# keras-team/keras-rs

Hardware: AMD Instinct MI355X
Metric: embedding lookups/sec + DCN fwd+bwd step time, 26-table DLRM batch 65 536 (higher is better)
Workload: dtype bf16; 1 GPU; C3 DLRM-small: 26 tables x 1000000 rows x 128 (bf16), global batch 65536, multi-hot ml_perf lengths (sum L = 214), uniform ids, DotInteraction(F=27) + 3 x FeatureCross(d=3456, projection=512), fused Adagrad on tables; global_batch=65536, parallelism=single GPU

## Files before the change

include/krs.h:

```cpp
#ifndef KRS_H_
#define KRS_H_

#include <stddef.h>
#include <stdint.h>

#ifdef __cplusplus
extern "C" {
#endif

#define KRS_VERSION 100

typedef enum krs_status {
  KRS_OK = 0,
  KRS_ERR_INVALID = -1,
  KRS_ERR_UNSUPPORTED = -2,
  KRS_ERR_LAUNCH = -3,
  KRS_ERR_WORKSPACE = -4
} krs_status;

typedef enum krs_dtype { KRS_F32 = 0, KRS_BF16 = 1 } krs_dtype;
typedef enum krs_itype { KRS_I32 = 0, KRS_I64 = 1 } krs_itype;

typedef enum krs_combiner { KRS_SUM = 0, KRS_MEAN = 1, KRS_SQRTN = 2 } krs_combiner;

// ... 87 lines not shown

int krs_embed_bag_bwd_fused_ftrl(const krs_table* tables, int n_tables,
                                 const krs_feature* feats, int n_feats,
                                 const float* weights, const float* bag_scale,
                                 const void* grad, int grad_dtype, int64_t grad_ld,
                                 int batch, int dim, int table_dtype, int64_t nnz,
                                 float learning_rate_power, float l1, float l2, float beta,
                                 const void* workspace, void* stream);

int krs_embed_bag_bwd_fused_adam_dyn(const krs_table* tables, int n_tables,
                                     const krs_feature* feats, int n_feats,
                                     const float* weights, const float* bag_scale,
                                     const void* grad, int grad_dtype, int64_t grad_ld,
                                     int batch, int dim, int table_dtype, int64_t nnz,
                                     float beta_1, float beta_2, float epsilon, const float* bias_correction_dev,
                                     const void* workspace, void* stream);

int krs_store_f32(void* dst, int64_t stride_bytes, const float* values_host, int count, void* stream);

int krs_embed_bag_bwd_sparse(const krs_feature* feats, int n_feats,
                             const float* weights, const float* bag_scale,
                             const void* grad, int grad_dtype, int64_t grad_ld,
                             int batch, int dim, int64_t nnz,
                             const void* workspace,
                             int64_t* unique_rows, float* row_grads, int64_t* n_unique,
                             void* stream);

typedef struct krs_gemm_epilogue {
  const float* bias;
  int32_t act;
  float diag_scale;
  const void* x0;
  const void* x;
  int64_t ldx;
  void* u_out;
  int64_t ldu;
  const void* r;
  int64_t ldr;
  float beta;
} krs_gemm_epilogue;

int krs_gemm(const void* a, int64_t lda, int a_is_km,
             const void* b, int64_t ldb, int b_is_nk,
             void* c, int64_t ldc,
             int64_t m, int64_t n, int64_t k,
             int in_dtype, int out_dtype,
             const krs_gemm_epilogue* epilogue,
             void* workspace, size_t workspace_bytes, void* stream);
size_t krs_gemm_workspace_bytes(int64_t m, int64_t n, int64_t k, int a_is_km);

size_t krs_gemm_cross_bwd_workspace_bytes(int64_t m, int64_t n);
int krs_gemm_cross_bwd(const void* a, int64_t lda, const void* bt, int64_t ldb,
                       const void* r, int64_t ldr, float beta,
                       void* g_out, int64_t ldg,
                       const void* x0, const void* u, void* dz, void* dx0, int64_t ld, int dx0_accumulate,
                       const void* u_upper, int fold_direct, float* dbias, int64_t m, int64_t n, int64_t k, int act, int dtype,
                       void* workspace, size_t workspace_bytes, void* stream);
int krs_gemm_dense_bwd(const void* a, int64_t lda, const void* bt, int64_t ldb, void* g_out, int64_t ldg,
                       const void* y, void* dz, int64_t ld, float* dbias, int64_t m, int64_t n, int64_t k, int act,
                       int dtype, void* workspace, size_t workspace_bytes, void* stream);
enum { KRS_CROSS_BWD_NONE = 0, KRS_CROSS_BWD_TWO_CALL = 1, KRS_CROSS_BWD_PP64 = 2, KRS_CROSS_BWD_PP256 = 3 };
int krs_gemm_cross_bwd_last_route(int* epilogue);

enum {
  KRS_GEMM_KERNEL_NONE = 0, KRS_GEMM_KERNEL_GENERIC = 1, KRS_GEMM_KERNEL_MFMA = 2, KRS_GEMM_KERNEL_GLDS = 3,
  KRS_GEMM_KERNEL_TN_GLDS = 4, KRS_GEMM_KERNEL_PP256 = 5, KRS_GEMM_KERNEL_PP256_KSTRIDED = 6, KRS_GEMM_KERNEL_PP64 = 7,
  KRS_GEMM_KERNEL_THIN = 8, KRS_GEMM_KERNEL_ROWDOT = 9, KRS_GEMM_KERNEL_SMALLK = 10
};
enum { KRS_GEMM_REDUCE_NONE = 0, KRS_GEMM_REDUCE_SCALAR = 1, KRS_GEMM_REDUCE_VEC4 = 2, KRS_GEMM_REDUCE_VEC8 = 3 };
typedef struct krs_gemm_route {
  int32_t kernel;
  int32_t splits;
  int32_t reduce;
  int32_t epilogue;
  int32_t ep_vec;
  int32_t thin_width;
  int32_t thin_is_a;
} krs_gemm_route;
int krs_gemm_last_route(krs_gemm_route* route);

enum { KRS_GEMM_OPT_PIPELINE = 0 };
int krs_gemm_set_option(int key, int value);

enum { KRS_EMBED_OPT_PLAN = 2, KRS_EMBED_OPT_HOTROWS = 3 };
int krs_embed_set_option(int key, int value);

size_t krs_colsum_workspace_bytes(int64_t m, int64_t n);
int krs_cross_epilogue_fwd(const void* u, const void* x0, const void* x, void* y,
                           int64_t m, int64_t n, int64_t ld, float diag_scale,
                           int dtype, void* stream);
int krs_cross_epilogue_bwd(const void* g, const void* u, const void* x0, const void* x,
                           void* du, void* dx0, int dx0_accumulate, void* dxd,
                           float* dbias,
                           int64_t m, int64_t n, int64_t ld, float diag_scale, int act,
                           int dtype, void* workspace, size_t workspace_bytes, void* stream);

int krs_cast_transpose(const void* src, int64_t rows, int64_t cols, int64_t ld_src, int src_dtype,
                       void* dst, int64_t ld_dst, void* dst_t, int64_t ld_dst_t, int dst_dtype,
                       void* stream);
int krs_cast_transpose_many(int count, const void* const* srcs, const int64_t* rows, const int64_t* cols,
                            int src_dtype, void* const* dsts, void* const* dst_ts, int dst_dtype, void* stream);

int krs_dense_act_bwd(const void* g, int64_t ld_g, const void* y, int64_t ld_y, void* dz, int64_t ld_dz,
                      float* dbias, int64_t m, int64_t n, int act, int dtype, void* workspace,
                      size_t workspace_bytes, void* stream);

int krs_dense_adagrad(float* const* params, const float* const* grads, float* const* accs,
                      const int64_t* sizes, int count, float lr, float eps, void* stream);

int krs_colsum(const void* a, int64_t lda, int64_t m, int64_t n, int dtype,
               float* out, void* workspace, size_t workspace_bytes, void* stream);

int krs_dot_interaction_fwd(const void* const* feats, const int64_t* ld, int n_feats,
                            int64_t batch, int dim, int dtype,
                            int self_interaction, int skip_gather,
                            void* out, int64_t out_ld, void* stream);
int krs_dot_interaction_bwd(const void* const* feats, const int64_t* ld, int n_feats,
                            int64_t batch, int dim, int dtype,
                            int self_interaction, int skip_gather,
                            const void* grad_out, int64_t grad_ld,
                            void* const* grad_feats, const int64_t* grad_feat_ld,
                            void* stream);
int krs_dot_interaction_bwd_accumulate(const void* const* feats, const int64_t* ld, int n_feats,
                                       int64_t batch, int dim, int dtype,
                                       int self_interaction, int skip_gather,
                                       const void* grad_out, int64_t grad_ld,
                                       void* const* grad_feats, const int64_t* grad_feat_ld,
                                       uint64_t accumulate_mask, void* stream);

size_t krs_mod_bucketize_workspace_bytes(int64_t nnz, int n_shards);
int krs_mod_bucketize(const void* ids, int id_type, int64_t nnz, int n_shards,
                      void* local_ids, int32_t* perm, int64_t* bucket_counts,
                      void* workspace, size_t workspace_bytes, void* stream);

#define KRS_BCE_MAX_BLOCKS 64
int krs_bce_fwd_bwd(const void* pred, int pred_dtype, const float* labels, int64_t n, float epsilon,
                    float grad_scale, float* loss, void* dpred, float* partials, void* stream);

typedef struct krs_shard_feature {
  int64_t ids_base;
  int64_t comp_off;
  int32_t hot;
  int32_t combiner;
  int32_t vocab;
  int32_t reserved;
} krs_shard_feature;

size_t krs_shard_route_workspace_bytes(int64_t nnz, int64_t n_bags, int n_shards);
int krs_shard_route(const krs_shard_feature* feats, const krs_shard_feature* feats_host, int n_feats,
                    const void* ids, int id_type, const void* offsets, int offset_type,
                    const float* weights, int64_t nnz, int batch, int n_shards, int emit_weights,
                    int32_t* packed, int32_t* seg_bag, int32_t* seg_grow, int32_t* bag_seg,
                    int64_t* counts, int32_t* err_flag,
                    void* workspace, size_t workspace_bytes, void* stream);
size_t krs_shard_unpack_workspace_bytes(int64_t total_segments);
int krs_shard_unpack(const int32_t* packed, int n_sources, const int64_t* lookups, const int64_t* segments,
                     int weighted, int32_t* rows, float* w, int32_t* offsets,
                     void* workspace, size_t workspace_bytes, void* stream);
int krs_shard_combine(const void* partials, const int32_t* bag_seg, int batch, int n_feats, int n_shards,
                      int dim, int dtype, void* out, int64_t out_ld, void* stream);
int64_t krs_shard_static_block_words(int64_t cap_lookups, int64_t cap_segments, int emit_weights);
int krs_shard_route_static(const krs_shard_feature* feats, const krs_shard_feature* feats_host, int n_feats,
                           const void* ids, int id_type, const void* offsets, int offset_type,
                           const float* weights, int64_t nnz, int batch, int n_shards, int emit_weights,
                           int64_t cap_lookups, int64_t cap_segments,
                           int32_t* packed, int32_t* seg_bag, int32_t* seg_grow, int32_t* bag_seg,
                           int64_t* counts, int32_t* err_flag,
// ... 73 lines not shown
```

keras_rs_amd/csrc/embed_bag_fwd.hip:

```cpp
#include <cstdlib>

#include "krs_common.h"

namespace krs {
namespace {

typedef uint32_t u32x4 __attribute__((ext_vector_type(4)));
typedef float f32x4 __attribute__((ext_vector_type(4)));
constexpr int NT = 2;

struct EmbedFwdParams {
  const krs_table* tables;
  const krs_feature* feats;
  int n_feats;
  const void* ids;
  int id64;
  const void* offsets;
  int off64;
  const float* weights;
  int batch;
  int dim;
  void* out;
  int64_t out_ld;
  float* bag_scale;
// ... 462 lines not shown
    sw2 = fmaf(w, w, sw2);
  }
  const int comb = ft.combiner;
  const float den = comb == KRS_MEAN ? sw : (comb == KRS_SQRTN ? sqrtf(sw2) : 1.0f);
  for (int c = sub; c < p.dim; c += lpr) {
    float acc = 0.0f;
    for (int64_t q = s; q < e; ++q) {
      const int64_t id = ld_index(p.ids, p.id64, q);
      if (id < 0 || id >= tb.vocab) {
        oob = 1;
        continue;
      }
      const float w = p.weights ? p.weights[q] : 1.0f;
      acc = fmaf(w, ld_elem(tb.weights, table_dtype, id * p.dim + c), acc);
    }
    if (comb != KRS_SUM) acc = den == 0.0f ? 0.0f : acc / den;
    st_elem(p.out, out_dtype, (int64_t)b * p.out_ld + ft.out_col + c, acc);
  }
  if (p.bag_scale && sub == 0)
    p.bag_scale[bag] = comb == KRS_SUM ? 1.0f : (den == 0.0f ? 0.0f : 1.0f / den);
  if (oob && p.err_flag && sub == 0) atomicOr(p.err_flag, KRS_FLAG_ID_OUT_OF_RANGE);
}

int g_hot_rows = 0;

template <typename TT, typename OT, int LPR>
int launch_vec(const EmbedFwdParams& p, bool one_hot, bool stream, hipStream_t st) {
  constexpr int G = 64 / LPR;
  if (one_hot) {
    if constexpr (sizeof(TT) == sizeof(OT)) {
      const bool rows_ok = p.n_feats <= kRowsMaxFeats &&
                           ((reinterpret_cast<uintptr_t>(p.out) | (uintptr_t)(p.out_ld * sizeof(OT))) & 15) == 0;
      if (rows_ok) {
        const int64_t blocks = ceil_div(ceil_div((int64_t)p.batch * p.n_feats, 64), 4);
        if (blocks > 0x7fffffffLL) return fail(KRS_ERR_UNSUPPORTED, "embed_bag_fwd: grid too large");
        hipLaunchKernelGGL((embed_gather_hot1_rows<TT, LPR, 16>), dim3((unsigned)blocks), dim3(256), 0, st, p);
        KRS_CHECK_LAUNCH("embed_gather_hot1_rows");
        return KRS_OK;
      }
    }
    const int64_t blocks = ceil_div(ceil_div(p.batch, 64) * p.n_feats, 4);
    if (blocks > 0x7fffffffLL) return fail(KRS_ERR_UNSUPPORTED, "embed_bag_fwd: grid too large");
    hipLaunchKernelGGL((embed_gather_hot1<TT, OT, LPR, 16>), dim3((unsigned)blocks), dim3(256), 0, st, p);
    KRS_CHECK_LAUNCH("embed_gather_hot1");
    return KRS_OK;
  }
  const int64_t waves_per_feat = ceil_div(p.batch, (int64_t)G * p.bpg);
  const int64_t blocks = ceil_div(waves_per_feat * p.n_feats, 4);
  if (blocks == 0) return KRS_OK;
  if (blocks > 0x7fffffffLL) return fail(KRS_ERR_UNSUPPORTED, "embed_bag_fwd: grid too large");
#define KRS_K1_LAUNCH(W, S) \
  hipLaunchKernelGGL((embed_bag_fwd_vec<TT, OT, LPR, W, S>), dim3((unsigned)blocks), dim3(256), 0, st, p)
  if constexpr (sizeof(TT) == 2 && sizeof(OT) == 2 && LPR == 16) {
    if (g_hot_rows > 0 && !p.weights && (int64_t)p.dim * 2 == LPR * 16) {
      if (g_hot_rows >= 128) {
        if (stream) hipLaunchKernelGGL((embed_bag_fwd_vec<TT, OT, LPR, false, true, 128>), dim3((unsigned)blocks), dim3(256), 0, st, p);
        else hipLaunchKernelGGL((embed_bag_fwd_vec<TT, OT, LPR, false, false, 128>), dim3((unsigned)blocks), dim3(256), 0, st, p);
      } else {
        if (stream) hipLaunchKernelGGL((embed_bag_fwd_vec<TT, OT, LPR, false, true, 64>), dim3((unsigned)blocks), dim3(256), 0, st, p);
        else hipLaunchKernelGGL((embed_bag_fwd_vec<TT, OT, LPR, false, false, 64>), dim3((unsigned)blocks), dim3(256), 0, st, p);
      }
      KRS_CHECK_LAUNCH("embed_bag_fwd_vec (hot rows in LDS)");
      return KRS_OK;
    }
  }
  if (p.weights) { if (stream) KRS_K1_LAUNCH(true, true); else KRS_K1_LAUNCH(true, false); }
  else { if (stream) KRS_K1_LAUNCH(false, true); else KRS_K1_LAUNCH(false, false); }
#undef KRS_K1_LAUNCH
  KRS_CHECK_LAUNCH("embed_bag_fwd_vec");
  return KRS_OK;
}

template <typename TT, typename OT>
int dispatch_lpr(const EmbedFwdParams& p, int row_pieces, bool one_hot, bool stream_mode, hipStream_t stream) {
  if (row_pieces <= 8) return launch_vec<TT, OT, 8>(p, one_hot, stream_mode, stream);
  if (row_pieces <= 16) return launch_vec<TT, OT, 16>(p, one_hot, stream_mode, stream);
  if (row_pieces <= 32) return launch_vec<TT, OT, 32>(p, one_hot, stream_mode, stream);
  return launch_vec<TT, OT, 64>(p, one_hot, stream_mode, stream);
}

}
}

namespace krs { extern int g_plan_variant; }

extern "C" int krs_embed_set_option(int key, int value) {
  if (key == KRS_EMBED_OPT_PLAN) {
    KRS_REQUIRE(value == 0 || value == 1, "krs_embed_set_option: plan variant must be 0 or 1");
    krs::g_plan_variant = value;
    return KRS_OK;
  }
  if (key == KRS_EMBED_OPT_HOTROWS) {
    KRS_REQUIRE(value == 0 || value == 64 || value == 128, "krs_embed_set_option: hot rows must be 0, 64 or 128");
    krs::g_hot_rows = value;
    return KRS_OK;
  }
  return krs::fail(KRS_ERR_INVALID, "krs_embed_set_option: unknown key %d", key);
}

extern "C" int krs_embed_bag_fwd(const krs_table* tables, const krs_feature* feats, int n_feats,
                                 const void* ids, int id_type, const void* offsets, int off_type,
                                 const float* weights, int64_t nnz, int batch, int dim,
                                 int table_dtype, void* out, int out_dtype, int64_t out_ld,
                                 float* bag_scale, int* err_flag, void* stream) {
  using namespace krs;
  KRS_REQUIRE(tables && feats && out, "embed_bag_fwd: null tables/feats/out");
  KRS_REQUIRE(ids || nnz == 0, "embed_bag_fwd: null ids");
  KRS_REQUIRE(n_feats >= 0 && batch >= 0 && dim > 0 && nnz >= 0, "embed_bag_fwd: negative size");
  KRS_REQUIRE((table_dtype == KRS_F32 || table_dtype == KRS_BF16) &&
                  (out_dtype == KRS_F32 || out_dtype == KRS_BF16),
              "embed_bag_fwd: bad dtype");
  KRS_REQUIRE((id_type == KRS_I32 || id_type == KRS_I64) && (off_type == KRS_I32 || off_type == KRS_I64),
              "embed_bag_fwd: bad index type");
  if (n_feats == 0 || batch == 0) return KRS_OK;
  hipStream_t st = reinterpret_cast<hipStream_t>(stream);

  EmbedFwdParams p;
  p.tables = tables; p.feats = feats; p.n_feats = n_feats;
  p.ids = ids; p.id64 = id_type == KRS_I64;
  p.offsets = offsets; p.off64 = off_type == KRS_I64;
  p.weights = weights; p.batch = batch; p.dim = dim;
  p.out = out; p.out_ld = out_ld; p.bag_scale = bag_scale; p.err_flag = err_flag;
  const int64_t n_bags = (int64_t)n_feats * batch;
  const int64_t mean_hot = nnz / n_bags > 0 ? nnz / n_bags : 1;
  int bpg = (int)(32 / mean_hot);
  p.bpg = bpg < 1 ? 1 : (bpg > 16 ? 16 : bpg);
  p.bpg = p.bpg < 1 ? 1 : (p.bpg > 16 ? 16 : p.bpg);

  const int64_t row_bytes = (int64_t)dim * (table_dtype == KRS_BF16 ? 2 : 4);
  if (row_bytes % 16 == 0 && row_bytes <= 1024) {
    const int pieces = (int)(row_bytes / 16);
    const bool one_hot = offsets == nullptr && weights == nullptr && nnz == n_bags;
    const bool stream_mode = nnz < 2 * n_bags;
    if (table_dtype == KRS_F32)
      return out_dtype == KRS_F32 ? dispatch_lpr<float, float>(p, pieces, one_hot, stream_mode, st)
                                  : dispatch_lpr<float, uint16_t>(p, pieces, one_hot, stream_mode, st);
    return out_dtype == KRS_F32 ? dispatch_lpr<uint16_t, float>(p, pieces, one_hot, stream_mode, st)
                                : dispatch_lpr<uint16_t, uint16_t>(p, pieces, one_hot, stream_mode, st);
  }
  int lpr = 1;
  while (lpr < dim && lpr < 64) lpr <<= 1;
  const int64_t blocks = ceil_div(n_bags, 256 / lpr);
  if (blocks > 0x7fffffffLL) return fail(KRS_ERR_UNSUPPORTED, "embed_bag_fwd: grid too large");
  hipLaunchKernelGGL(embed_bag_fwd_generic, dim3((unsigned)blocks), dim3(256), 0, st, p, table_dtype,
                     out_dtype, lpr);
  KRS_CHECK_LAUNCH("embed_bag_fwd_generic");
  return KRS_OK;
}
```

keras_rs_amd/csrc/embed_bag_plan.hip:

```cpp
#include <algorithm>

#include "krs_bag_plan.h"

namespace krs {
int g_plan_variant = 0;
namespace {

namespace rs {
constexpr int kHistThreads = 256, kHistItems = kTile / kHistThreads;
constexpr int kThreads = 512, kWaves = kThreads / 64, kItems = kTile / kThreads;
constexpr int kGenFeats = 256;

struct Gen {
  const krs_table* tables;
  const krs_feature* feats;
  int n_feats;
  const void* ids;
  int id64;
  int batch;
  int* err_flag;
};

struct alignas(16) GenLds {
  uint32_t base[kGenFeats + 1];
  uint32_t hot[kGenFeats];
  uint32_t row_base[kGenFeats];
  uint32_t vocab[kGenFeats];
};
__device__ __forceinline__ void load_gen(const Gen& gen, int64_t nnz, GenLds& g, int n_threads) {
  for (int i = threadIdx.x; i <= gen.n_feats; i += n_threads) {
    if (i < gen.n_feats) {
      const krs_feature ft = gen.feats[i];
      const krs_table tb = gen.tables[ft.table];
      g.base[i] = (uint32_t)ft.ids_base;
      g.hot[i] = (uint32_t)ft.hot;
      g.row_base[i] = (uint32_t)tb.row_base;
      g.vocab[i] = (uint32_t)tb.vocab;
    } else {
      g.base[i] = (uint32_t)nnz;
    }
  }
}
__device__ __forceinline__ int gen_feature(const GenLds& g, int n_feats, uint32_t q) {
  int lo = 0, hi = n_feats;
  while (hi - lo > 1) {
    const int mid = (lo + hi) >> 1;
    if (g.base[mid] <= q) lo = mid; else hi = mid;
  }
  return lo;
}
__device__ __forceinline__ uint64_t gen_value(const Gen& gen, const GenLds& g, int f, uint32_t q) {
  const uint32_t bag = (uint32_t)f * (uint32_t)gen.batch + (q - g.base[f]) / g.hot[f];
  return ((uint64_t)bag << 32) | (uint64_t)q;
}
__device__ __forceinline__ bool generate(const Gen& gen, const GenLds& g, uint32_t q, uint32_t& key, uint64_t& val) {
  const int f = gen_feature(g, gen.n_feats, q);
  const int64_t id = ld_index(gen.ids, gen.id64, q);
  const bool valid = id >= 0 && id < (int64_t)g.vocab[f];
  key = valid ? g.row_base[f] + (uint32_t)id : kInvalidKey;
  val = gen_value(gen, g, f, q);
  return valid;
}

__device__ __forceinline__ int digit_of(uint32_t key, int shift, int bins) { return (int)((key >> shift) & (bins - 1)); }

__device__ __forceinline__ void hist_zero(int (&h)[kMaxBins], int bins) {
  for (int i = threadIdx.x; i < bins; i += kHistThreads) h[i] = 0;
}
__device__ __forceinline__ void hist_add(int (&h)[kMaxBins], uint32_t key, int shift, int bins) {
  atomicAdd(&h[digit_of(key, shift, bins)], 1);
}
__device__ __forceinline__ void hist_finish(const int (&h)[kMaxBins], int bins, int32_t* col, int64_t stride, bool bad,
                                            int* err_flag) {
  if (bad && err_flag) atomicOr(err_flag, KRS_FLAG_ID_OUT_OF_RANGE);
  __syncthreads();
  for (int i = threadIdx.x; i < bins; i += kHistThreads) col[(int64_t)i * stride] = h[i];
}

template <typename V>
struct alignas(16) TileLds {
  uint16_t cnt[kWaves][kMaxBins];
  uint16_t tile_excl[kMaxBins];
  int gbase[kMaxBins];
  uint32_t skey[kTile];
  V sval[kTile];
  int wtot[kWaves];
};
template <typename V>
__device__ __forceinline__ void zero_counts(TileLds<V>& s) {
  for (int i = threadIdx.x; i < kWaves * kMaxBins; i += kThreads) (&s.cnt[0][0])[i] = 0;
}
__device__ __forceinline__ int ballot_rank(uint32_t key, bool live, int shift, int bits, volatile uint16_t* mine,
                                           int lane) {
  const int d = digit_of(key, shift, 1 << bits);
  unsigned long long peers = __ballot(live);
  for (int b = 0; b < bits; ++b) {
    const unsigned long long m = __ballot((d >> b) & 1);
    peers &= ((d >> b) & 1) ? m : ~m;
  }
  int r = 0, c = 0;
  if (live) {
    r = __popcll(peers & ((1ULL << lane) - 1ULL));
    const int leader = __ffsll((long long)peers) - 1;
    if (lane == leader) {
      c = mine[d];
      mine[d] = (uint16_t)(c + __popcll(peers));
    }
    c = __shfl(c, leader, 64);
  }
  __builtin_amdgcn_wave_barrier();
  return c + r;
}
template <typename V>
__device__ __forceinline__ void digit_bases(TileLds<V>& s, int bins, const int32_t* col, int64_t stride) {
  const int lane = threadIdx.x & 63, wave = threadIdx.x >> 6;
  __syncthreads();
  int tot[2], run = 0;
#pragma unroll
  for (int k = 0; k < 2; ++k) {
    const int i = threadIdx.x * 2 + k;
    tot[k] = 0;
    if (i < bins)
      for (int w = 0; w < kWaves; ++w) tot[k] += s.cnt[w][i];
    run += tot[k];
  }
  int x = run;
#pragma unroll
  for (int o = 1; o < 64; o <<= 1) {
    const int y = __shfl_up(x, o, 64);
    if (lane >= o) x += y;
  }
  if (lane == 63) s.wtot[wave] = x;
  __syncthreads();
  int excl = x - run;
  for (int w = 0; w < wave; ++w) excl += s.wtot[w];
#pragma unroll
  for (int k = 0; k < 2; ++k) {
    const int i = threadIdx.x * 2 + k;
    if (i < bins) {
      s.tile_excl[i] = (uint16_t)excl;
      s.gbase[i] = col[(int64_t)i * stride];
      int o = excl;
      for (int w = 0; w < kWaves; ++w) {
        const int t = s.cnt[w][i];
        s.cnt[w][i] = (uint16_t)o;
        o += t;
      }
      excl += tot[k];
    }
  }
  __syncthreads();
}
template <typename V>
__device__ __forceinline__ void stage_tile(TileLds<V>& s, const uint32_t (&key)[kItems], const V (&val)[kItems],
                                           const int (&rank)[kItems], int64_t first, int64_t end, int shift, int bins) {
  const int wave = threadIdx.x >> 6;
#pragma unroll
  for (int it = 0; it < kItems; ++it) {
    if (first + it * 64 < end) {
      const int lp = s.cnt[wave][digit_of(key[it], shift, bins)] + rank[it];
      s.skey[lp] = key[it];
      s.sval[lp] = val[it];
    }
  }
  __syncthreads();
}
template <typename V>
__device__ __forceinline__ int out_slot(const TileLds<V>& s, int i, int d) {
  return s.gbase[d] + (i - (int)s.tile_excl[d]);
}

struct Pass {
  const uint32_t* keys_in;
  const uint64_t* vals_in;
  uint32_t* keys_out;
  uint64_t* vals_out;
  int32_t* counts;
  int64_t nnz;
  int n_tiles;
  int shift, bits;
  Gen gen;
};

template <bool GEN>
__global__ __launch_bounds__(kHistThreads) void hist_kernel(const Pass p) {
  __shared__ int h[kMaxBins];
  __shared__ GenLds g;
  const int bins = 1 << p.bits;
  hist_zero(h, bins);
  if constexpr (GEN) load_gen(p.gen, p.nnz, g, kHistThreads);
  __syncthreads();
  const int64_t base = (int64_t)blockIdx.x * kTile;
  bool bad = false;
  for (int it = 0; it < kHistItems; ++it) {
    const int64_t q = base + it * kHistThreads + threadIdx.x;
    if (q < p.nnz) {
      uint32_t key;
      if constexpr (GEN) {
        uint64_t v;
        bad |= !generate(p.gen, g, (uint32_t)q, key, v);
      } else {
        key = p.keys_in[q];
      }
      hist_add(h, key, p.shift, bins);
    }
  }
  hist_finish(h, bins, p.counts + blockIdx.x, p.n_tiles, bad, p.gen.err_flag);
}

template <bool GEN>
__global__ __launch_bounds__(kThreads) void scatter_kernel(const Pass p) {
  __shared__ TileLds<uint64_t> s;
  __shared__ GenLds g;
  const int bins = 1 << p.bits;
  zero_counts(s);
  if constexpr (GEN) load_gen(p.gen, p.nnz, g, kThreads);
  __syncthreads();
  const int lane = threadIdx.x & 63, wave = threadIdx.x >> 6;
  const int64_t tile0 = (int64_t)blockIdx.x * kTile;
  const int64_t first = tile0 + (int64_t)wave * (kTile / kWaves) + lane;
  uint32_t key[kItems];
  uint64_t val[kItems];
  int rank[kItems];
#pragma unroll
  for (int it = 0; it < kItems; ++it) {
    const int64_t q = first + it * 64;
    const bool live = q < p.nnz;
    key[it] = kInvalidKey;
    val[it] = 0;
    if (live) {
      if constexpr (GEN) {
        generate(p.gen, g, (uint32_t)q, key[it], val[it]);
      } else {
        key[it] = p.keys_in[q];
        val[it] = p.vals_in[q];
      }
    }
    rank[it] = ballot_rank(key[it], live, p.shift, p.bits, s.cnt[wave], lane);
  }
  digit_bases(s, bins, p.counts + blockIdx.x, p.n_tiles);
  stage_tile(s, key, val, rank, first, p.nnz, p.shift, bins);
  const int n_here = (int)min<int64_t>(kTile, p.nnz - tile0);
#pragma unroll
  for (int it = 0; it < kItems; ++it) {
    const int i = it * kThreads + threadIdx.x;
    if (i < n_here) {
      const uint32_t k = s.skey[i];
      const int pos = out_slot(s, i, digit_of(k, p.shift, bins));
      p.keys_out[pos] = k;
      p.vals_out[pos] = s.sval[i];
    }
  }
}

struct Seg {
  int n;
  uint32_t lookup_start[kMaxProb + 1];
  uint32_t tile_start[kMaxProb + 1];
  uint32_t row_base[kMaxProb];
};
struct SegPass {
  const uint32_t* keys_in;
  const uint32_t* pos_in;
  uint32_t* keys_out;
  uint32_t* pos_out;
  uint64_t* vals_out;
  int32_t* counts;
  int64_t nnz;
  int shift, bits, key_bits;
  Gen gen;
  Seg seg;
};
struct SegTile {
  int pr;
  int64_t t0, end;
  int32_t* col;
  uint32_t stride;
};
__device__ __forceinline__ SegTile seg_tile(const SegPass& p, uint32_t tile) {
  const Seg& sg = p.seg;
  int lo = 0, hi = sg.n;
  while (hi - lo > 1) {
    const int mid = (lo + hi) >> 1;
    if (sg.tile_start[mid] <= tile) lo = mid; else hi = mid;
  }
  SegTile t;
  t.pr = lo;
  const uint32_t tl = tile - sg.tile_start[lo];
  t.stride = sg.tile_start[lo + 1] - sg.tile_start[lo];
  t.t0 = (int64_t)sg.lookup_start[lo] + (int64_t)tl * kTile;
  t.end = min<int64_t>(t.t0 + kTile, sg.lookup_start[lo + 1]);
  t.col = p.counts + ((int64_t)1 << p.bits) * sg.tile_start[lo] + tl;
  return t;
}
template <int ITEMS, int STRIDE>
__device__ __forceinline__ bool seg_first_keys(const SegPass& p, const GenLds& g, const SegTile& t, int64_t first,
                                               uint32_t (&key)[ITEMS], uint32_t (&pos)[ITEMS]) {
  int64_t idv[ITEMS];
#pragma unroll
  for (int it = 0; it < ITEMS; ++it) idv[it] = ld_index(p.gen.ids, p.gen.id64, min<int64_t>(first + it * STRIDE, t.end - 1));
  const int f_lo = gen_feature(g, p.gen.n_feats, (uint32_t)t.t0), f_hi = gen_feature(g, p.gen.n_feats, (uint32_t)(t.end - 1));
  bool bad = false;
#pragma unroll
  for (int it = 0; it < ITEMS; ++it) {
    const int64_t q = min<int64_t>(first + it * STRIDE, t.end - 1);
    const int f = f_lo == f_hi ? f_lo : gen_feature(g, p.gen.n_feats, (uint32_t)q);
    const bool valid = idv[it] >= 0 && idv[it] < (int64_t)g.vocab[f];
    key[it] = valid ? (uint32_t)idv[it] : (1u << p.key_bits) - 1u;
    pos[it] = (uint32_t)q;
    bad = bad || (!valid && first + it * STRIDE < t.end);
  }
  return bad;
}

template <bool FIRST>
__global__ __launch_bounds__(kHistThreads) void hist_seg_kernel(const SegPass p) {
  __shared__ int h[kMaxBins];
  __shared__ GenLds g;
  const int bins = 1 << p.bits;
  hist_zero(h, bins);
  if constexpr (FIRST) load_gen(p.gen, p.nnz, g, kHistThreads);
  __syncthreads();
  const SegTile t = seg_tile(p, blockIdx.x);
  const int64_t first = t.t0 + threadIdx.x;
  bool bad = false;
  uint32_t key[kHistItems];
  if constexpr (FIRST) {
    uint32_t pos[kHistItems];
    bad = seg_first_keys<kHistItems, kHistThreads>(p, g, t, first, key, pos);
  } else {
#pragma unroll
    for (int it = 0; it < kHistItems; ++it) key[it] = p.keys_in[min<int64_t>(first + it * kHistThreads, t.end - 1)];
  }
#pragma unroll
  for (int it = 0; it < kHistItems; ++it)
    if (first + it * kHistThreads < t.end) hist_add(h, key[it], p.shift, bins);
  hist_finish(h, bins, t.col, t.stride, bad, p.gen.err_flag);
}

template <bool FIRST, bool LAST>
__global__ __launch_bounds__(kThreads) void scatter_seg_kernel(const SegPass p) {
  __shared__ TileLds<uint32_t> s;
  __shared__ GenLds g;
  const int bins = 1 << p.bits;
  zero_counts(s);
  if constexpr (FIRST || LAST) load_gen(p.gen, p.nnz, g, kThreads);
  __syncthreads();
  const int lane = threadIdx.x & 63, wave = threadIdx.x >> 6;
  const SegTile t = seg_tile(p, blockIdx.x);
  const int64_t first = t.t0 + (int64_t)wave * (kTile / kWaves) + lane;
  uint32_t key[kItems], pos[kItems];
  int rank[kItems];
  if constexpr (FIRST) {
    seg_first_keys<kItems, 64>(p, g, t, first, key, pos);
  } else {
#pragma unroll
    for (int it = 0; it < kItems; ++it) {
      const int64_t q = min<int64_t>(first + it * 64, t.end - 1);
      key[it] = p.keys_in[q];
      pos[it] = p.pos_in[q];
    }
  }
#pragma unroll
  for (int it = 0; it < kItems; ++it) {
    const bool live = first + it * 64 < t.end;
    if (!live) { key[it] = 0xffffffffu; pos[it] = 0; }
    rank[it] = ballot_rank(key[it], live, p.shift, p.bits, s.cnt[wave], lane);
  }
  digit_bases(s, bins, t.col, t.stride);
  stage_tile(s, key, pos, rank, first, t.end, p.shift, bins);
  const int n_here = (int)(t.end - t.t0);
  const uint32_t sentinel = (1u << p.key_bits) - 1u, rb = p.seg.row_base[t.pr];
  int pf_lo = 0, pf_hi = 1;
  if constexpr (LAST) {
    pf_lo = gen_feature(g, p.gen.n_feats, p.seg.lookup_start[t.pr]);
    pf_hi = gen_feature(g, p.gen.n_feats, p.seg.lookup_start[t.pr + 1] - 1);
  }
#pragma unroll
  for (int it = 0; it < kItems; ++it) {
    const int i = it * kThreads + threadIdx.x;
    if (i < n_here) {
      const uint32_t k = s.skey[i], q = s.sval[i];
      const int o = out_slot(s, i, digit_of(k, p.shift, bins));
      if constexpr (LAST) {
        const int f = pf_lo == pf_hi ? pf_lo : gen_feature(g, p.gen.n_feats, q);
        p.keys_out[o] = k == sentinel ? kInvalidKey : rb + k;
        p.vals_out[o] = gen_value(p.gen, g, f, q);
      } else {
        p.keys_out[o] = k;
        p.pos_out[o] = q;
      }
    }
  }
}

inline unsigned key_bits(int64_t n) {
  unsigned bits = 1;
  while (bits < 32 && (1ULL << bits) <= (uint64_t)n) ++bits;
  return bits;
}
struct Schedule {
  int passes;
  int bits[4], shift[4];
};
inline Schedule pass_schedule(unsigned bits) {
  Schedule s;
  s.passes = (int)((bits + kMaxBits - 1) / kMaxBits);
  unsigned done = 0;
  for (int ps = 0; ps < s.passes; ++ps) {
    s.bits[ps] = (int)((bits - done + (s.passes - ps) - 1) / (s.passes - ps));
    s.shift[ps] = (int)done;
    done += (unsigned)s.bits[ps];
  }
  return s;
}
inline Gen make_gen(const krs_table* tables, const krs_feature* feats, int n_feats, const void* ids, int id_type,
                    int batch, int* err_flag) {
  Gen g;
  g.tables = tables; g.feats = feats; g.n_feats = n_feats; g.ids = ids;
  g.id64 = id_type == KRS_I64; g.batch = batch; g.err_flag = err_flag;
  return g;
}
}

struct KeyParams {
  const krs_table* tables;
  const krs_feature* feats;
  int n_feats;
  const void* ids;
  int id64;
  const void* offsets;
  int off64;
  int batch;
  uint32_t* keys;
  uint64_t* vals;
  int* err_flag;
};

__global__ __launch_bounds__(256) void bag_keys_kernel(const KeyParams p) {
  const int64_t bag = (int64_t)blockIdx.x * 16 + (threadIdx.x >> 4);
  const int sub = threadIdx.x & 15;
  if (bag >= (int64_t)p.n_feats * p.batch) return;
  const int f = (int)(bag / p.batch);
  const int b = (int)(bag - (int64_t)f * p.batch);
  const krs_feature ft = p.feats[f];
  const krs_table tb = p.tables[ft.table];
  int64_t s, e;
  if (p.offsets) {
    s = ld_index(p.offsets, p.off64, bag);
    e = ld_index(p.offsets, p.off64, bag + 1);
  } else {
// ... 46 lines not shown
  int c = __popc(seg_head_mask(keys, nnz, (int64_t)blockIdx.x * kSegTile + threadIdx.x * kSegItems));
  for (int o = 32; o; o >>= 1) c += __shfl_down(c, o, 64);
  if ((threadIdx.x & 63) == 0) atomicAdd(&total, c);
  __syncthreads();
  if (threadIdx.x == 0) block_heads[blockIdx.x] = total;
}
__global__ __launch_bounds__(256) void seg_emit_kernel(const uint32_t* keys, int64_t nnz, const int32_t* block_off,
                                                       uint32_t* seg_start, uint32_t* n_seg) {
  __shared__ int wsum[4];
  const int64_t t0 = (int64_t)blockIdx.x * kSegTile + threadIdx.x * kSegItems;
  const uint32_t mask = seg_head_mask(keys, nnz, t0);
  const int c = __popc(mask), lane = threadIdx.x & 63, wave = threadIdx.x >> 6;
  int x = c;
#pragma unroll
  for (int o = 1; o < 64; o <<= 1) {
    const int y = __shfl_up(x, o, 64);
    if (lane >= o) x += y;
  }
  if (lane == 63) wsum[wave] = x;
  __syncthreads();
  uint32_t off = (uint32_t)block_off[blockIdx.x] + (uint32_t)(x - c);
  for (int w = 0; w < wave; ++w) off += (uint32_t)wsum[w];
  uint32_t m = mask;
  while (m) {
    const int k = __ffs(m) - 1;
    m &= m - 1;
    seg_start[off++] = (uint32_t)(t0 + k);
  }
  if (t0 < nnz && t0 + kSegItems >= nnz) *n_seg = off;
}
__global__ void long_list_kernel(const uint32_t* seg_start, const uint32_t* n_seg, int64_t nnz, uint32_t* counters,
                                 LongItem* items, MultiSeg* multi) {
  const int64_t u = (int64_t)blockIdx.x * blockDim.x + threadIdx.x;
  const uint32_t ns = *n_seg;
  if (u >= ns) return;
  const int64_t e = u + 1 < ns ? (int64_t)seg_start[u + 1] : nnz;
  const int64_t len = e - (int64_t)seg_start[u];
  if (len <= kLongSeg) return;
  const uint32_t nch = (uint32_t)((len + kChunk - 1) / kChunk);
  const uint32_t base = atomicAdd(counters, nch);
  uint32_t pb = 0xffffffffu;
  if (nch > 1) {
    pb = atomicAdd(counters + 1, nch);
    multi[atomicAdd(counters + 2, 1u)] = MultiSeg{(uint32_t)u, pb, nch};
  }
  for (uint32_t c = 0; c < nch; ++c) items[base + c] = LongItem{(uint32_t)u, c, nch > 1 ? pb + c : 0xffffffffu};
}

bool plan_sort_by_table(const PlanLayout& l, const rs::Temp& tmp, const rs::Gen& gen, const krs_table* tables_host,
                        int n_tables, const krs_feature* feats_host, int64_t nnz, hipStream_t st) {
  if (!tables_host || !feats_host || gen.n_feats > rs::kGenFeats || n_tables <= 0) return false;
  rs::SegPass sp;
  rs::Seg& sg = sp.seg;
  sg.n = 0;
  int64_t pos = 0, max_vocab = 0;
  int prev_table = -1;
  for (int f = 0; f < gen.n_feats; ++f) {
    const krs_feature& ft = feats_host[f];
    if (ft.hot < 1 || ft.ids_base != pos || ft.table < prev_table || ft.table >= n_tables) return false;
    if (ft.table != prev_table) {
      if (sg.n == rs::kMaxProb) return false;
      const krs_table& tb = tables_host[ft.table];
      if (prev_table >= 0 && tb.row_base < tables_host[prev_table].row_base + tables_host[prev_table].vocab) return false;
      sg.lookup_start[sg.n] = (uint32_t)pos;
      sg.row_base[sg.n] = (uint32_t)tb.row_base;
      max_vocab = std::max<int64_t>(max_vocab, tb.vocab);
      ++sg.n;
      prev_table = ft.table;
    }
    pos += (int64_t)gen.batch * ft.hot;
  }
  if (pos != nnz || sg.n == 0) return false;
  sg.lookup_start[sg.n] = (uint32_t)nnz;
  uint32_t tiles = 0;
  for (int i = 0; i < sg.n; ++i) {
    sg.tile_start[i] = tiles;
    tiles += (uint32_t)ceil_div((int64_t)sg.lookup_start[i + 1] - sg.lookup_start[i], rs::kTile);
  }
  sg.tile_start[sg.n] = tiles;
  if (tiles == 0) return false;
  const unsigned bits = rs::key_bits(max_vocab);
  if (bits > 31) return false;
  const rs::Schedule sch = rs::pass_schedule(bits);
  sp.counts = tmp.counts; sp.nnz = nnz; sp.key_bits = (int)bits;
  sp.gen = gen;
  uint32_t* k0 = l.keys_in; uint32_t* q0 = reinterpret_cast<uint32_t*>(l.vals_in);
  uint32_t* k1 = l.keys_sorted; uint32_t* q1 = reinterpret_cast<uint32_t*>(l.vals_sorted);
  for (int ps = 0; ps < sch.passes; ++ps) {
    const bool first = ps == 0, last = ps == sch.passes - 1;
    sp.bits = sch.bits[ps];
    sp.shift = sch.shift[ps];
    const bool out_is_i0 = ((sch.passes - 2 - ps) % 2) == 0;
    const bool in_is_i0 = ((sch.passes - 1 - ps) % 2) == 0;
    sp.keys_in = first ? nullptr : (in_is_i0 ? k0 : k1);
    sp.pos_in = first ? nullptr : (in_is_i0 ? q0 : q1);
    sp.keys_out = last ? l.keys_sorted : (out_is_i0 ? k0 : k1);
    sp.pos_out = last ? nullptr : (out_is_i0 ? q0 : q1);
    sp.vals_out = last ? l.vals_sorted : nullptr;
    if (first) hipLaunchKernelGGL(rs::hist_seg_kernel<true>, dim3(tiles), dim3(rs::kHistThreads), 0, st, sp);
    else hipLaunchKernelGGL(rs::hist_seg_kernel<false>, dim3(tiles), dim3(rs::kHistThreads), 0, st, sp);
    scan::exclusive(tmp.counts, tmp.counts, (int64_t)(1 << sp.bits) * tiles, tmp.sums, nullptr, st);
    if (first && last) hipLaunchKernelGGL((rs::scatter_seg_kernel<true, true>), dim3(tiles), dim3(rs::kThreads), 0, st, sp);
    else if (first) hipLaunchKernelGGL((rs::scatter_seg_kernel<true, false>), dim3(tiles), dim3(rs::kThreads), 0, st, sp);
    else if (last) hipLaunchKernelGGL((rs::scatter_seg_kernel<false, true>), dim3(tiles), dim3(rs::kThreads), 0, st, sp);
    else hipLaunchKernelGGL((rs::scatter_seg_kernel<false, false>), dim3(tiles), dim3(rs::kThreads), 0, st, sp);
  }
  return true;
}

int plan_sort_global(const PlanLayout& l, const rs::Temp& tmp, const rs::Gen& gen, const void* offsets, int off_type,
                     int64_t nnz, int64_t total_rows, hipStream_t st) {
  const rs::Schedule sch = rs::pass_schedule(rs::key_bits(total_rows));
  const bool gen_first = offsets == nullptr && gen.n_feats <= rs::kGenFeats;
  bool to_sorted = (sch.passes % 2) == 1;
  if (!gen_first) {
    KeyParams kp;
    kp.tables = gen.tables; kp.feats = gen.feats; kp.n_feats = gen.n_feats; kp.ids = gen.ids; kp.id64 = gen.id64;
    kp.offsets = offsets; kp.off64 = off_type == KRS_I64; kp.batch = gen.batch; kp.err_flag = gen.err_flag;
    kp.keys = to_sorted ? l.keys_in : l.keys_sorted;
    kp.vals = to_sorted ? l.vals_in : l.vals_sorted;
    const int64_t n_bags = (int64_t)gen.n_feats * gen.batch;
    KRS_HIP(hipMemsetAsync(kp.keys, 0xff, (size_t)nnz * sizeof(uint32_t), st));
    hipLaunchKernelGGL(bag_keys_kernel, dim3((unsigned)ceil_div(n_bags, 16)), dim3(256), 0, st, kp);
    KRS_CHECK_LAUNCH("bag_keys_kernel");
  }
  rs::Pass p;
  p.nnz = nnz;
  p.n_tiles = (int)ceil_div(nnz, rs::kTile);
  p.counts = tmp.counts;
  p.gen = gen;
  for (int ps = 0; ps < sch.passes; ++ps) {
    p.bits = sch.bits[ps];
    p.shift = sch.shift[ps];
    const bool generating = gen_first && ps == 0;
    p.keys_in = generating ? nullptr : (to_sorted ? l.keys_in : l.keys_sorted);
    p.vals_in = generating ? nullptr : (to_sorted ? l.vals_in : l.vals_sorted);
    p.keys_out = to_sorted ? l.keys_sorted : l.keys_in;
    p.vals_out = to_sorted ? l.vals_sorted : l.vals_in;
    if (generating) hipLaunchKernelGGL(rs::hist_kernel<true>, dim3(p.n_tiles), dim3(rs::kHistThreads), 0, st, p);
    else hipLaunchKernelGGL(rs::hist_kernel<false>, dim3(p.n_tiles), dim3(rs::kHistThreads), 0, st, p);
    scan::exclusive(tmp.counts, tmp.counts, (int64_t)(1 << p.bits) * p.n_tiles, tmp.sums, nullptr, st);
    if (generating) hipLaunchKernelGGL(rs::scatter_kernel<true>, dim3(p.n_tiles), dim3(rs::kThreads), 0, st, p);
    else hipLaunchKernelGGL(rs::scatter_kernel<false>, dim3(p.n_tiles), dim3(rs::kThreads), 0, st, p);
    to_sorted = !to_sorted;
  }
  return KRS_OK;
}

int plan_impl(const krs_table* tables, const krs_table* tables_host, int n_tables, const krs_feature* feats,
              const krs_feature* feats_host, int n_feats, const void* ids, int id_type, const void* offsets,
              int off_type, int batch, int64_t nnz, int64_t total_rows, void* workspace, size_t workspace_bytes,
              int* err_flag, void* stream) {
  KRS_REQUIRE(tables && feats && (ids || nnz == 0), "embed_bag_bwd_plan: null argument");
  KRS_REQUIRE(n_feats > 0 && batch > 0 && nnz >= 0, "embed_bag_bwd_plan: bad sizes");
  KRS_REQUIRE(total_rows > 0 && total_rows < 0xffffffffLL, "embed_bag_bwd_plan: total_rows must fit 32-bit keys");
  KRS_REQUIRE(nnz < 0x7fffffffLL && (int64_t)n_feats * batch < 0xffffffffLL,
              "embed_bag_bwd_plan: nnz must stay below 2^31 and the bag count below 2^32");
  if (nnz == 0) return KRS_OK;
  KRS_REQUIRE(workspace, "embed_bag_bwd_plan: null workspace");
  const PlanLayout l = plan_layout(workspace, nnz, true);
  if (workspace_bytes < l.total_bytes)
    return fail(KRS_ERR_WORKSPACE, "embed_bag_bwd_plan: workspace %zu < %zu bytes", workspace_bytes, l.total_bytes);
  hipStream_t st = reinterpret_cast<hipStream_t>(stream);
  const rs::Temp tmp = rs::carve_temp(l.temp, nnz);
  const rs::Gen gen = rs::make_gen(tables, feats, n_feats, ids, id_type, batch, err_flag);
  const bool by_table = offsets == nullptr && g_plan_variant == 0 &&
                        plan_sort_by_table(l, tmp, gen, tables_host, n_tables, feats_host, nnz, st);
  if (!by_table)
    if (int rc = plan_sort_global(l, tmp, gen, offsets, off_type, nnz, total_rows, st)) return rc;
  KRS_CHECK_LAUNCH("embed_bag_bwd_plan: radix sort");
  const unsigned nb = (unsigned)ceil_div(nnz, 256);
  const unsigned nsb = (unsigned)ceil_div(nnz, kSegTile);
  hipLaunchKernelGGL(seg_count_kernel, dim3(nsb), dim3(256), 0, st, l.keys_sorted, nnz, tmp.sums2);
  hipLaunchKernelGGL(scan::block_kernel, dim3(1), dim3(1024), 0, st, tmp.sums2, (int64_t)nsb, (int64_t*)nullptr);
  hipLaunchKernelGGL(seg_emit_kernel, dim3(nsb), dim3(256), 0, st, l.keys_sorted, nnz, tmp.sums2, l.seg_start, l.n_seg);
  KRS_CHECK_LAUNCH("seg_emit_kernel");
  KRS_HIP(hipMemsetAsync(l.n_long, 0, 3 * sizeof(uint32_t), st));
  KRS_HIP(hipMemsetAsync(l.sort_mode, by_table ? 1 : 0, sizeof(uint32_t), st));
  hipLaunchKernelGGL(long_list_kernel, dim3(nb), dim3(256), 0, st, l.seg_start, l.n_seg, nnz, l.n_long, l.long_list,
                     l.multi_list);
  KRS_CHECK_LAUNCH("long_list_kernel");
  return KRS_OK;
}

}
}

using namespace krs;

extern "C" size_t krs_embed_bag_bwd_workspace_bytes(int64_t nnz) {
  if (nnz < 0) return 0;
  return plan_layout(nullptr, nnz, true).total_bytes;
}

extern "C" int krs_embed_bag_bwd_plan(const krs_table* tables, const krs_feature* feats, int n_feats,
                                      const void* ids, int id_type, const void* offsets, int off_type,
                                      int batch, int64_t nnz, int64_t total_rows, void* workspace,
                                      size_t workspace_bytes, int* err_flag, void* stream) {
  return plan_impl(tables, nullptr, 0, feats, nullptr, n_feats, ids, id_type, offsets, off_type, batch, nnz, total_rows,
                   workspace, workspace_bytes, err_flag, stream);
}

extern "C" int krs_embed_bag_bwd_plan_tables(const krs_table* tables, const krs_table* tables_host, int n_tables,
                                             const krs_feature* feats, const krs_feature* feats_host, int n_feats,
                                             const void* ids, int id_type, int batch, int64_t nnz, int64_t total_rows,
                                             void* workspace, size_t workspace_bytes, int* err_flag, void* stream) {
  KRS_REQUIRE(tables_host && feats_host && n_tables > 0, "embed_bag_bwd_plan_tables: null host descriptors");
  return plan_impl(tables, tables_host, n_tables, feats, feats_host, n_feats, ids, id_type, nullptr, KRS_I32, batch, nnz,
                   total_rows, workspace, workspace_bytes, err_flag, stream);
}
```

Baseline: 1.476 billion lookups/s.

## Rank radix-sort digits with LDS atomic counts and remap tiles across XCDs

Adds a new within-wave digit ranking for the backward-plan radix sort. It uses wave-scoped atomic adds on packed 16-bit LDS counters and resolves only colliding digits with per-leader ballots, falling back to the bitwise ballot ranking when collisions are many. This is meant to cut the per-bit ballot loop cost in the scatter kernels. It also remaps block indices so consecutive tiles are spread in groups of eight, likely to match the MI355X chiplet (XCD) scheduling, at the cost of some idle padded blocks. A new option selects the ranking mode, and the new hybrid mode is the default.

```diff
diff --git a/include/krs.h b/include/krs.h
--- a/include/krs.h
+++ b/include/krs.h
@@ -193,7 +193,7 @@
 enum { KRS_GEMM_OPT_PIPELINE = 0 };
 int krs_gemm_set_option(int key, int value);
 
-enum { KRS_EMBED_OPT_PLAN = 2, KRS_EMBED_OPT_HOTROWS = 3 };
+enum { KRS_EMBED_OPT_PLAN = 2, KRS_EMBED_OPT_HOTROWS = 3, KRS_EMBED_OPT_RANK = 4 };
 int krs_embed_set_option(int key, int value);
 
 size_t krs_colsum_workspace_bytes(int64_t m, int64_t n);
diff --git a/keras_rs_amd/csrc/embed_bag_fwd.hip b/keras_rs_amd/csrc/embed_bag_fwd.hip
--- a/keras_rs_amd/csrc/embed_bag_fwd.hip
+++ b/keras_rs_amd/csrc/embed_bag_fwd.hip
@@ -568,12 +568,17 @@
 }
 }
 
-namespace krs { extern int g_plan_variant; }
+namespace krs { extern int g_plan_variant, g_rank_mode; }
 
 extern "C" int krs_embed_set_option(int key, int value) {
   if (key == KRS_EMBED_OPT_PLAN) {
     KRS_REQUIRE(value == 0 || value == 1, "krs_embed_set_option: plan variant must be 0 or 1");
     krs::g_plan_variant = value;
+    return KRS_OK;
+  }
+  if (key == KRS_EMBED_OPT_RANK) {
+    KRS_REQUIRE(value >= 0 && value <= 2, "krs_embed_set_option: rank mode must be 0, 1 or 2");
+    krs::g_rank_mode = value;
     return KRS_OK;
   }
   if (key == KRS_EMBED_OPT_HOTROWS) {
diff --git a/keras_rs_amd/csrc/embed_bag_plan.hip b/keras_rs_amd/csrc/embed_bag_plan.hip
--- a/keras_rs_amd/csrc/embed_bag_plan.hip
+++ b/keras_rs_amd/csrc/embed_bag_plan.hip
@@ -4,6 +4,7 @@
 
 namespace krs {
 int g_plan_variant = 0;
+int g_rank_mode = 0;
 namespace {
 
 namespace rs {
@@ -64,6 +65,9 @@
 
 __device__ __forceinline__ int digit_of(uint32_t key, int shift, int bins) { return (int)((key >> shift) & (bins - 1)); }
 
+__device__ __forceinline__ uint32_t tile_of_block(uint32_t b, uint32_t tiles) { return (b & 7) * ((tiles + 7) / 8) + (b >> 3); }
+inline unsigned tile_grid(unsigned tiles) { return (tiles + 7) / 8 * 8; }
+
 __device__ __forceinline__ void hist_zero(int (&h)[kMaxBins], int bins) {
   for (int i = threadIdx.x; i < bins; i += kHistThreads) h[i] = 0;
 }
@@ -90,14 +94,18 @@
 __device__ __forceinline__ void zero_counts(TileLds<V>& s) {
   for (int i = threadIdx.x; i < kWaves * kMaxBins; i += kThreads) (&s.cnt[0][0])[i] = 0;
 }
-__device__ __forceinline__ int ballot_rank(uint32_t key, bool live, int shift, int bits, volatile uint16_t* mine,
-                                           int lane) {
-  const int d = digit_of(key, shift, 1 << bits);
+__device__ __forceinline__ unsigned long long digit_peers(int d, bool live, int bits) {
   unsigned long long peers = __ballot(live);
   for (int b = 0; b < bits; ++b) {
     const unsigned long long m = __ballot((d >> b) & 1);
     peers &= ((d >> b) & 1) ? m : ~m;
   }
+  return peers;
+}
+__device__ __forceinline__ int ballot_rank(uint32_t key, bool live, int shift, int bits, volatile uint16_t* mine,
+                                           int lane) {
+  const int d = digit_of(key, shift, 1 << bits);
+  const unsigned long long peers = digit_peers(d, live, bits);
   int r = 0, c = 0;
   if (live) {
     r = __popcll(peers & ((1ULL << lane) - 1ULL));
@@ -110,6 +118,55 @@
   }
   __builtin_amdgcn_wave_barrier();
   return c + r;
+}
+typedef uint32_t __attribute__((may_alias)) cnt_word;
+__device__ __forceinline__ void count_rank(const uint32_t (&key)[kItems], int64_t first, int64_t end, int shift, int bits,
+                                           bool fallback, uint16_t* mine, int lane, int (&rank)[kItems]) {
+  cnt_word* word = reinterpret_cast<cnt_word*>(mine);
+  uint32_t before[kItems], after[kItems];
+#pragma unroll
+  for (int it = 0; it < kItems; ++it) {
+    const int d = digit_of(key[it], shift, 1 << bits);
+    const bool live = first + it * 64 < end;
+    cnt_word* w = word + (d >> 1);
+    before[it] = __hip_atomic_load(w, __ATOMIC_RELAXED, __HIP_MEMORY_SCOPE_WAVEFRONT);
+    __builtin_amdgcn_wave_barrier();
+    __hip_atomic_fetch_add(w, live ? 1u << (16 * (d & 1)) : 0u, __ATOMIC_RELAXED, __HIP_MEMORY_SCOPE_WAVEFRONT);
+    __builtin_amdgcn_wave_barrier();
+    after[it] = __hip_atomic_load(w, __ATOMIC_RELAXED, __HIP_MEMORY_SCOPE_WAVEFRONT);
+    __builtin_amdgcn_wave_barrier();
+  }
+  const unsigned long long below = (1ULL << lane) - 1ULL;
+#pragma unroll
+  for (int it = 0; it < kItems; ++it) {
+    const int d = digit_of(key[it], shift, 1 << bits);
+    const bool live = first + it * 64 < end;
+    const int c = (int)((before[it] >> (16 * (d & 1))) & 0xffffu);
+    const int n = (int)((after[it] >> (16 * (d & 1))) & 0xffffu) - c;
+    int r = c;
+    unsigned long long pend = __ballot(live && n > 1);
+    if (fallback && __popcll(pend) / 2 > bits) {
+      r = c + __popcll(digit_peers(d, live, bits) & below);
+    } else {
+      while (pend) {
+        const int leader = __ffsll((long long)pend) - 1;
+        const int dl = __builtin_amdgcn_readlane(d, leader);
+        const unsigned long long peers = __ballot(live && d == dl);
+        if (d == dl) r = c + __popcll(peers & below);
+        pend &= ~peers;
+      }
+    }
+    rank[it] = live ? r : 0;
+  }
+}
+__device__ __forceinline__ void rank_keys(const uint32_t (&key)[kItems], int64_t first, int64_t end, int shift, int bits,
+                                          int mode, uint16_t* mine, int lane, int (&rank)[kItems]) {
+  if (mode == 1) {
+#pragma unroll
+    for (int it = 0; it < kItems; ++it) rank[it] = ballot_rank(key[it], first + it * 64 < end, shift, bits, mine, lane);
+  } else {
+    count_rank(key, first, end, shift, bits, mode == 0, mine, lane, rank);
+  }
 }
 template <typename V>
 __device__ __forceinline__ void digit_bases(TileLds<V>& s, int bins, const int32_t* col, int64_t stride) {
@@ -179,6 +236,7 @@
   int64_t nnz;
   int n_tiles;
   int shift, bits;
+  int rank;
   Gen gen;
 };
 
@@ -186,11 +244,13 @@
 __global__ __launch_bounds__(kHistThreads) void hist_kernel(const Pass p) {
   __shared__ int h[kMaxBins];
   __shared__ GenLds g;
+  const uint32_t tile = tile_of_block(blockIdx.x, p.n_tiles);
+  if (tile >= (uint32_t)p.n_tiles) return;
   const int bins = 1 << p.bits;
   hist_zero(h, bins);
   if constexpr (GEN) load_gen(p.gen, p.nnz, g, kHistThreads);
   __syncthreads();
-  const int64_t base = (int64_t)blockIdx.x * kTile;
+  const int64_t base = (int64_t)tile * kTile;
   bool bad = false;
   for (int it = 0; it < kHistItems; ++it) {
     const int64_t q = base + it * kHistThreads + threadIdx.x;
@@ -205,19 +265,21 @@
       hist_add(h, key, p.shift, bins);
     }
   }
-  hist_finish(h, bins, p.counts + blockIdx.x, p.n_tiles, bad, p.gen.err_flag);
+  hist_finish(h, bins, p.counts + tile, p.n_tiles, bad, p.gen.err_flag);
 }
 
 template <bool GEN>
 __global__ __launch_bounds__(kThreads) void scatter_kernel(const Pass p) {
   __shared__ TileLds<uint64_t> s;
   __shared__ GenLds g;
+  const uint32_t tile = tile_of_block(blockIdx.x, p.n_tiles);
+  if (tile >= (uint32_t)p.n_tiles) return;
   const int bins = 1 << p.bits;
   zero_counts(s);
   if constexpr (GEN) load_gen(p.gen, p.nnz, g, kThreads);
   __syncthreads();
   const int lane = threadIdx.x & 63, wave = threadIdx.x >> 6;
-  const int64_t tile0 = (int64_t)blockIdx.x * kTile;
+  const int64_t tile0 = (int64_t)tile * kTile;
   const int64_t first = tile0 + (int64_t)wave * (kTile / kWaves) + lane;
   uint32_t key[kItems];
   uint64_t val[kItems];
@@ -236,9 +298,9 @@
         val[it] = p.vals_in[q];
       }
     }
-    rank[it] = ballot_rank(key[it], live, p.shift, p.bits, s.cnt[wave], lane);
-  }
-  digit_bases(s, bins, p.counts + blockIdx.x, p.n_tiles);
+  }
+  rank_keys(key, first, p.nnz, p.shift, p.bits, p.rank, s.cnt[wave], lane, rank);
+  digit_bases(s, bins, p.counts + tile, p.n_tiles);
   stage_tile(s, key, val, rank, first, p.nnz, p.shift, bins);
   const int n_here = (int)min<int64_t>(kTile, p.nnz - tile0);
 #pragma unroll
@@ -268,6 +330,7 @@
   int32_t* counts;
   int64_t nnz;
   int shift, bits, key_bits;
+  int rank;
   Gen gen;
   Seg seg;
 };
@@ -317,11 +380,13 @@
 __global__ __launch_bounds__(kHistThreads) void hist_seg_kernel(const SegPass p) {
   __shared__ int h[kMaxBins];
   __shared__ GenLds g;
+  const uint32_t tile = tile_of_block(blockIdx.x, p.seg.tile_start[p.seg.n]);
+  if (tile >= p.seg.tile_start[p.seg.n]) return;
   const int bins = 1 << p.bits;
   hist_zero(h, bins);
   if constexpr (FIRST) load_gen(p.gen, p.nnz, g, kHistThreads);
   __syncthreads();
-  const SegTile t = seg_tile(p, blockIdx.x);
+  const SegTile t = seg_tile(p, tile);
   const int64_t first = t.t0 + threadIdx.x;
   bool bad = false;
   uint32_t key[kHistItems];
@@ -342,12 +407,14 @@
 __global__ __launch_bounds__(kThreads) void scatter_seg_kernel(const SegPass p) {
   __shared__ TileLds<uint32_t> s;
   __shared__ GenLds g;
+  const uint32_t tile = tile_of_block(blockIdx.x, p.seg.tile_start[p.seg.n]);
+  if (tile >= p.seg.tile_start[p.seg.n]) return;
   const int bins = 1 << p.bits;
   zero_counts(s);
   if constexpr (FIRST || LAST) load_gen(p.gen, p.nnz, g, kThreads);
   __syncthreads();
   const int lane = threadIdx.x & 63, wave = threadIdx.x >> 6;
-  const SegTile t = seg_tile(p, blockIdx.x);
+  const SegTile t = seg_tile(p, tile);
   const int64_t first = t.t0 + (int64_t)wave * (kTile / kWaves) + lane;
   uint32_t key[kItems], pos[kItems];
   int rank[kItems];
@@ -365,8 +432,8 @@
   for (int it = 0; it < kItems; ++it) {
     const bool live = first + it * 64 < t.end;
     if (!live) { key[it] = 0xffffffffu; pos[it] = 0; }
-    rank[it] = ballot_rank(key[it], live, p.shift, p.bits, s.cnt[wave], lane);
-  }
+  }
+  rank_keys(key, first, t.end, p.shift, p.bits, p.rank, s.cnt[wave], lane, rank);
   digit_bases(s, bins, t.col, t.stride);
   stage_tile(s, key, pos, rank, first, t.end, p.shift, bins);
   const int n_here = (int)(t.end - t.t0);
@@ -579,7 +646,7 @@
   const unsigned bits = rs::key_bits(max_vocab);
   if (bits > 31) return false;
   const rs::Schedule sch = rs::pass_schedule(bits);
-  sp.counts = tmp.counts; sp.nnz = nnz; sp.key_bits = (int)bits;
+  sp.counts = tmp.counts; sp.nnz = nnz; sp.key_bits = (int)bits; sp.rank = g_rank_mode;
   sp.gen = gen;
   uint32_t* k0 = l.keys_in; uint32_t* q0 = reinterpret_cast<uint32_t*>(l.vals_in);
   uint32_t* k1 = l.keys_sorted; uint32_t* q1 = reinterpret_cast<uint32_t*>(l.vals_sorted);
@@ -594,13 +661,13 @@
     sp.keys_out = last ? l.keys_sorted : (out_is_i0 ? k0 : k1);
     sp.pos_out = last ? nullptr : (out_is_i0 ? q0 : q1);
     sp.vals_out = last ? l.vals_sorted : nullptr;
-    if (first) hipLaunchKernelGGL(rs::hist_seg_kernel<true>, dim3(tiles), dim3(rs::kHistThreads), 0, st, sp);
-    else hipLaunchKernelGGL(rs::hist_seg_kernel<false>, dim3(tiles), dim3(rs::kHistThreads), 0, st, sp);
+    if (first) hipLaunchKernelGGL(rs::hist_seg_kernel<true>, dim3(rs::tile_grid(tiles)), dim3(rs::kHistThreads), 0, st, sp);
+    else hipLaunchKernelGGL(rs::hist_seg_kernel<false>, dim3(rs::tile_grid(tiles)), dim3(rs::kHistThreads), 0, st, sp);
     scan::exclusive(tmp.counts, tmp.counts, (int64_t)(1 << sp.bits) * tiles, tmp.sums, nullptr, st);
-    if (first && last) hipLaunchKernelGGL((rs::scatter_seg_kernel<true, true>), dim3(tiles), dim3(rs::kThreads), 0, st, sp);
-    else if (first) hipLaunchKernelGGL((rs::scatter_seg_kernel<true, false>), dim3(tiles), dim3(rs::kThreads), 0, st, sp);
-    else if (last) hipLaunchKernelGGL((rs::scatter_seg_kernel<false, true>), dim3(tiles), dim3(rs::kThreads), 0, st, sp);
-    else hipLaunchKernelGGL((rs::scatter_seg_kernel<false, false>), dim3(tiles), dim3(rs::kThreads), 0, st, sp);
+    if (first && last) hipLaunchKernelGGL((rs::scatter_seg_kernel<true, true>), dim3(rs::tile_grid(tiles)), dim3(rs::kThreads), 0, st, sp);
+    else if (first) hipLaunchKernelGGL((rs::scatter_seg_kernel<true, false>), dim3(rs::tile_grid(tiles)), dim3(rs::kThreads), 0, st, sp);
+    else if (last) hipLaunchKernelGGL((rs::scatter_seg_kernel<false, true>), dim3(rs::tile_grid(tiles)), dim3(rs::kThreads), 0, st, sp);
+    else hipLaunchKernelGGL((rs::scatter_seg_kernel<false, false>), dim3(rs::tile_grid(tiles)), dim3(rs::kThreads), 0, st, sp);
   }
   return true;
 }
@@ -625,6 +692,7 @@
   p.nnz = nnz;
   p.n_tiles = (int)ceil_div(nnz, rs::kTile);
   p.counts = tmp.counts;
+  p.rank = g_rank_mode;
   p.gen = gen;
   for (int ps = 0; ps < sch.passes; ++ps) {
     p.bits = sch.bits[ps];
@@ -634,11 +702,11 @@
     p.vals_in = generating ? nullptr : (to_sorted ? l.vals_in : l.vals_sorted);
     p.keys_out = to_sorted ? l.keys_sorted : l.keys_in;
     p.vals_out = to_sorted ? l.vals_sorted : l.vals_in;
-    if (generating) hipLaunchKernelGGL(rs::hist_kernel<true>, dim3(p.n_tiles), dim3(rs::kHistThreads), 0, st, p);
-    else hipLaunchKernelGGL(rs::hist_kernel<false>, dim3(p.n_tiles), dim3(rs::kHistThreads), 0, st, p);
+    if (generating) hipLaunchKernelGGL(rs::hist_kernel<true>, dim3(rs::tile_grid((unsigned)p.n_tiles)), dim3(rs::kHistThreads), 0, st, p);
+    else hipLaunchKernelGGL(rs::hist_kernel<false>, dim3(rs::tile_grid((unsigned)p.n_tiles)), dim3(rs::kHistThreads), 0, st, p);
     scan::exclusive(tmp.counts, tmp.counts, (int64_t)(1 << p.bits) * p.n_tiles, tmp.sums, nullptr, st);
-    if (generating) hipLaunchKernelGGL(rs::scatter_kernel<true>, dim3(p.n_tiles), dim3(rs::kThreads), 0, st, p);
-    else hipLaunchKernelGGL(rs::scatter_kernel<false>, dim3(p.n_tiles), dim3(rs::kThreads), 0, st, p);
+    if (generating) hipLaunchKernelGGL(rs::scatter_kernel<true>, dim3(rs::tile_grid((unsigned)p.n_tiles)), dim3(rs::kThreads), 0, st, p);
+    else hipLaunchKernelGGL(rs::scatter_kernel<false>, dim3(rs::tile_grid((unsigned)p.n_tiles)), dim3(rs::kThreads), 0, st, p);
     to_sorted = !to_sorted;
   }
   return KRS_OK;
```

Result: faster. 1.492 billion lookups/s (median of 6 runs) (+1.0%).
